# bittremieux/falcon

Hardware: AMD Instinct MI355X
Metric: spectra clustered/sec @1/2/4/8 GPU; cosine-kernel HBM GB/s vs roofline (higher is better)
Workload: dtype f32; 1 GPU; one dataset of 1000000 synthetic spectra (1000000 per GPU; charges 2+3; precursor m/z 400-1200), low_dim=400, n_neighbors=64, n_neighbors_ann=128, n_probe=16, eps=0.1, precursor_tol=20ppm, mz_interval=1.0, batch_size=32768; exchange=none, parallelism=1 GPU

## Files before the change

### falcon_amd/csrc/common.h

```cpp
#pragma once
#include <hip/hip_runtime.h>
#include <stdint.h>
#include <stdio.h>
#include <string.h>
#include <string>
#include <vector>
#include "../../include/falcon_hip.h"

namespace fal {

void set_error(const char* fmt, ...);

#define FAL_CHECK_HIP(expr)                                                          \
    do {                                                                             \
        hipError_t _e = (expr);                                                      \
        if (_e != hipSuccess) {                                                      \
            fal::set_error("%s:%d: %s failed: %s", __FILE__, __LINE__, #expr,        \
                           hipGetErrorString(_e));                                   \
            return (_e == hipErrorOutOfMemory) ? FAL_ENOMEM : FAL_EHIP;              \
        }                                                                            \
    } while (0)

#define FAL_REQUIRE(cond, code, ...)                                                 \
    do {                                                                             \
        if (!(cond)) {                                                               \
            fal::set_error(__VA_ARGS__);                                             \
            return (code);                                                           \
        }                                                                            \
    } while (0)

#define FAL_TRY(expr)                                                                \
    do {                                                                             \
        int _r = (expr);                                                             \
        if (_r != FAL_OK) return _r;                                                 \
    } while (0)

constexpr int kNumStages = 9;
constexpr int kNumSlots = 37;
enum Stage { ST_VECTORIZE = 0, ST_BUILD = 1, ST_COARSE = 2, ST_SCAN = 3, ST_SELECT = 4,
             ST_FILTER = 5, ST_DBSCAN = 6, ST_TAIL = 7,
             ST_KERNEL = 8 };

struct Scratch {
    void* ptr = nullptr;
    size_t cap = 0;
};

}

struct fal_ctx {
    int device = -1;
    hipStream_t stream = nullptr;
    bool own_stream = false;
    void* pinned = nullptr;
    size_t pinned_cap = 0;
    int pinned_reserve(size_t bytes, void** out);
    unsigned char* arena = nullptr;
    size_t arena_off = 0;
    int upload(void* dst, const void* src, size_t bytes);
    int num_cus = 256;
    int persistent_wgs = 256;
    bool timing = false;
    struct StageTimer {
        std::vector<std::pair<hipEvent_t, hipEvent_t>> ev;
        size_t used = 0;
    } timers[fal::kNumStages];
    fal::Scratch scratch[fal::kNumSlots];
    int32_t* fb_host = nullptr;
    int32_t* zero_dev = nullptr;
    int64_t counters[10] = {0, 0, 0, 0, 0, 0, 0, 0, 0, 0};

    struct PoolBlock { void* ptr; size_t cap; bool used; };
    std::vector<PoolBlock> pool;
    int pool_alloc(size_t bytes, void** out);
    void pool_free(void* ptr);

    bool debug_poison = false;
    int call_depth = 0;
    uint64_t call_epoch = 1;
    uint64_t slot_epoch[fal::kNumSlots] = {};
    uint32_t slot_gen[fal::kNumSlots] = {};
    std::vector<void*> retired;
    std::vector<bool> retired_held;
    void release_retired();
    int reserve(int slot, size_t bytes, void** out);
    void release(int slot) { slot_epoch[slot] = 0; }
    void stage_reset(int stage);
    int stage_begin(int stage, hipEvent_t* stop_out, hipStream_t on = nullptr);
    int stage_end(hipEvent_t stop, hipStream_t on = nullptr);
};

namespace fal {

struct StageScope {
    fal_ctx* c;
    hipEvent_t stop = nullptr;
    bool on;
    hipStream_t s;
    StageScope(fal_ctx* ctx, int stage, hipStream_t stream = nullptr, bool enable = true)
        : c(ctx), on(ctx->timing && enable), s(stream) {
        if (on) c->stage_begin(stage, &stop, s);
    }
    ~StageScope() {
        if (on && stop) c->stage_end(stop, s);
    }
};

struct CallScope {
    fal_ctx* c;
    explicit CallScope(fal_ctx* ctx) : c(ctx) {
        if (c && c->call_depth++ == 0) {
            ++c->call_epoch;
            if (!c->retired.empty()) c->release_retired();
        }
    }
    ~CallScope() {
        if (c) --c->call_depth;
    }
};

static inline int64_t ceil_div(int64_t a, int64_t b) { return (a + b - 1) / b; }
// ... 89 lines not shown
```

### falcon_amd/csrc/ivf.h

```cpp
#pragma once
#include <vector>
#include "common.h"

namespace fal {
constexpr int kSparseW = 64;
constexpr uint16_t kColPad = 0xFFFF;
constexpr uint16_t kColDense = 0xFFFE;

enum { SLOT_JOBS = 0, SLOT_SIMS = 1, SLOT_PROBES = 2, SLOT_PROBE_SIM = 3, SLOT_QOFF = 4, SLOT_JOBS2 = 5,
       SLOT_MISC = 6, SLOT_MISC2 = 7, SLOT_SORT = 8, SLOT_SORT2 = 9, SLOT_TAIL = 10, SLOT_TAIL2 = 11,
       SLOT_TAIL3 = 12, SLOT_TAIL4 = 13, SLOT_DB = 14, SLOT_DB2 = 15, SLOT_DB3 = 16, SLOT_FIN = 17, SLOT_FIN2 = 18,
       SLOT_FIN3 = 19, SLOT_INV = 20, SLOT_INVCNT = 21, SLOT_SIMS2 = 22, SLOT_TILEJOB = 23, SLOT_FUSED = 24, SLOT_FUSED2 = 25, SLOT_FUSED3 = 26, SLOT_JOBS3 = 27, SLOT_WIN = 28, SLOT_CURSORS = 29, SLOT_ITEMS = 30,
       SLOT_EXACT = 31, SLOT_EXACT2 = 32, SLOT_EXACT3 = 33, SLOT_EXACT4 = 34, SLOT_EXACT5 = 35, SLOT_EXACT6 = 36 };
int launch_exclusive_scan(fal_ctx* ctx, const int64_t* in, int64_t n, int64_t* out);
}
struct fal_ivf;
namespace fal {
int ivf_ensure_xl(fal_ctx* ctx, const fal_ivf* ivf);
}

struct fal_ivf {
    fal_ctx* ctx = nullptr;
    int64_t n = 0;
    int d = 0;
    const float* X = nullptr;
    const float* Xl = nullptr;
    float* Xl_owned = nullptr;
    const void* X16 = nullptr;
    int x16_planes = 0;
    const void* Xpre = nullptr;
    int rows_signed = 0;
    int rows_f16 = 0;
    int32_t* neg_dev = nullptr;
    const void* X16pre = nullptr;
    int32_t* pos_of_row = nullptr;
    int ckeys_stride = 0;
    uint16_t* ckeys = nullptr;
    std::vector<int64_t> bucket_off;
    std::vector<int32_t> n_list;
    std::vector<int64_t> list_base;
    int64_t total_lists = 0;
    int n_ivf_buckets = 0;
    int64_t ivf_waves = 0;
    float* centroids = nullptr;
    int32_t* assign = nullptr;
    int32_t* perm = nullptr;
    uint16_t* sp_cols = nullptr;
    float* sp_vals = nullptr;
    uint16_t* sq16 = nullptr;
    int rows_many = 0;
    int64_t* list_off = nullptr;
    int64_t* counts = nullptr;
    void* bk_dev = nullptr;
};
```

### falcon_amd/csrc/scan.h

```cpp
#pragma once
#include "common.h"
#include "simtile.h"

namespace fal {

enum { EPI_STORE = 0, EPI_ARGMAX = 1 };
enum { MODE_DENSE = 0, MODE_IVF = 1 };

constexpr size_t kSimsSlack = 2048;

struct SelectArgs {
    const float* sims;
    int64_t sims_base;
    int k;
    float* out_sim;
    int32_t* out_idx;
    const DenseJob* jobs;
    int n_jobs;
    int64_t tile_begin;
    const int32_t* tile_job;
    int ids_are_rows;
    int n_probe;
    const int32_t* probes;
    const int64_t* list_off;
    const int64_t* q_sim_off;
    const int32_t* perm;
    const float* f_pmz;
    const float* f_rt;
    double f_tol, f_rt_tol;
    int f_is_da;
    int f_keep;
    int32_t* nb_idx;
    float* nb_dist;
    int32_t* nb_count;
};

bool dense4_supports(int d);
int launch_dense4(fal_ctx* ctx, const float* X, int d, const DenseJob* jobs, const DenseJob* jobs_host, int n_jobs, float* sims,
                  int64_t sims_base);
bool dense4ab_supports(int d);
int launch_dense4ab(fal_ctx* ctx, const float* X, int d, const DenseJob* jobs, const DenseJob* jobs_host, int n_jobs, float* sims,
                    int64_t sims_base);
int launch_dense_tiny4(fal_ctx* ctx, const float* X, int d, const DenseJob* jobs, int n_jobs, float* sims, int64_t sims_base);
int launch_flat_exact_small(fal_ctx* ctx, const float* X, int d, const DenseJob* jobs, int n_jobs, float* sims, int64_t sims_base);
int launch_dense(fal_ctx* ctx, int stage, int epi, const float* Q, const float* Cm, int d, const DenseJob* jobs,
                 int n_jobs, int64_t tile_begin, int64_t n_tiles, float* sims, int64_t sims_base, int32_t* assign,
                 int64_t xcd_list_tiles = 0);
constexpr int kAssignSeg = 2048;
constexpr int kAssignGroup = 128;
constexpr int kAssignMergeLists = 2048;
struct AssignJob {
    int64_t row0;
    int64_t cent0;
    int32_t nrows;
    int32_t ncent;
    int32_t id_base;
    int32_t part0;
};
int launch_assign(fal_ctx* ctx, int stage, const float* X, const float* centroids, int d, const AssignJob* jobs, int64_t n_jobs,
                  int64_t n_wave_jobs, int64_t n, unsigned long long* keys, int32_t* assign);
bool assign16_supports(int d);
int launch_cvt_f16(fal_ctx* ctx, const float* in, void* out, int64_t count);
int launch_assign16(fal_ctx* ctx, int stage, const void* X16, const float* X, const void* C16, const float* Cn, int d,
                    const AssignJob* jobs, int64_t n_single, int64_t n_merge, int64_t n_group, int64_t n_rows, int32_t* assign,
                    uint16_t* ckeys = nullptr, int ckeys_stride = 0, const uint16_t* sp_cols = nullptr,
                    const float* sp_vals = nullptr, int merge_max_lists = 4 * kAssignGroup, int64_t merge_rows = 0);
struct ListScanArgs {
    const float* Xl;
    int d;
    const int64_t* list_off;
    const int64_t* inv_off;
    const int64_t* ltile_off;
    int group_shift;
    const int32_t* inv_q;
    const int64_t* inv_dest;
    int64_t list_begin, list_end;
    int64_t tile_begin, n_tiles_max;
    float* sims;
    int64_t sims_base;
    float* sink;
};
int launch_list_scan(fal_ctx* ctx, const ListScanArgs& a);
int launch_select(fal_ctx* ctx, int stage, int mode, const SelectArgs& a, int64_t n_blocks, hipStream_t on = nullptr);
int launch_scan16(fal_ctx* ctx, int planes, const void* Xs, int d, const DenseJob* jobs, int n_jobs, int64_t list_tiles,
                  float* sims, int64_t sims_base, float* sink);

}
```

### falcon_amd/csrc/scan.hip

```cpp
#include <math.h>
#include <stdlib.h>
#include <string.h>
#include <algorithm>
#include "common.h"
#include "simtile.h"
#include "scan.h"
#include "select.h"
#include "ivf.h"

namespace fal {

template <int DH4, int EPI>
__global__ __launch_bounds__(64, 1) void dense_kernel(
    const float* __restrict__ Q, const float* __restrict__ Cm, int d, const DenseJob* __restrict__ jobs,
    int n_jobs, int64_t tile_begin, int64_t n_tiles, float* __restrict__ sims, int64_t sims_base,
    int32_t* __restrict__ assign, int xcd_lists, int symmetric) {
    DenseJob job;
    int lt;
    int ji = 0;
    if (xcd_lists) {
        if (!find_job_xcd(jobs, n_jobs, blockIdx.x, &ji, &lt)) return;
        job = jobs[ji];
    } else {
        const int64_t per_xcd = (n_tiles + 7) / 8;
        const int64_t lt_all = (int64_t)(blockIdx.x & 7) * per_xcd + (blockIdx.x >> 3);
        if ((blockIdx.x >> 3) >= per_xcd || lt_all >= n_tiles) return;
        const int64_t t = tile_begin + lt_all;
        job = jobs[find_job(jobs, n_jobs, t)];
        lt = (int)(t - job.tile0);
    }
    const int lane = threadIdx.x, r = lane & 31, h = lane >> 5;
    const int nq_t = min(32, job.nq - 32 * lt);
    const int dh = d >> 1, dh4 = dh >> 2;

    float q[DH4 * 4];
    {
        const int64_t qrow = job.q_row0 + 32 * (int64_t)lt + min(r, nq_t - 1);
        load_half_row<DH4>(q, Q + qrow * d + (int64_t)h * dh, dh4);
    }
    float best = -INFINITY;
    int bestc = 0x7fffffff;
    const int nc = job.nc;
    float* out = nullptr;
    const int ncp = (nc + 31) & ~31;
    if (EPI == EPI_STORE) out = sims + (job.obase - sims_base) + (int64_t)(32 * lt) * ncp + r;

    const int c_first = (EPI == EPI_STORE && symmetric) ? 32 * lt : 0;
    float* outT = nullptr;
    if (EPI == EPI_STORE && symmetric) outT = sims + (job.obase - sims_base) + (int64_t)r * ncp + 32 * lt + 4 * h;
    const int c_last = ((nc - 1) >> 5) << 5;
    constexpr bool kDown = EPI == EPI_STORE;
    const int c_begin = kDown ? c_last : 0, c_step = kDown ? -32 : 32;
    const int n_chunks = (c_last - c_first) / 32 + 1;
    CandStream<DH4> cs;
    const float* cur = Cm + (job.c_row0 + min(c_begin + r, nc - 1)) * d + (int64_t)h * dh;
    cs.prime(cur, dh4);
    f32x16 prev;
    int prev_c0 = c_begin;
#pragma unroll
    for (int i = 0; i < 16; ++i) prev[i] = (EPI == EPI_STORE) ? 0.f : -INFINITY;
    auto epilogue = [&]() {
        if (EPI == EPI_STORE) {
#pragma unroll
            for (int i = 0; i < 16; ++i) out[mfma32_row(i, h) * ncp + prev_c0] = prev[i];
            if (symmetric) {
                float* t = outT + (int64_t)prev_c0 * ncp;
#pragma unroll
                for (int g = 0; g < 4; ++g)
                    *reinterpret_cast<float4*>(t + 8 * g) = make_float4(prev[4 * g], prev[4 * g + 1], prev[4 * g + 2], prev[4 * g + 3]);
                __builtin_amdgcn_sched_group_barrier(0x040, 20, 0);
            } else {
                __builtin_amdgcn_sched_group_barrier(0x040, 16, 0);
            }
        } else {
#pragma unroll
            for (int i = 0; i < 16; ++i) {
                const int c = prev_c0 + mfma32_row(i, h);
                const float s = prev[i];
                if (c < nc && s > best) {
                    best = s;
                    bestc = c;
                }
            }
        }
    };
    for (int ci = 0, c0 = c_begin; ci < n_chunks; ++ci, c0 += c_step) {
        const float* nxt = Cm + (job.c_row0 + min(max(c0 + c_step, 0) + r, nc - 1)) * d + (int64_t)h * dh;
        const f32x16 acc = (EPI == EPI_STORE) ? cs.template dot<true>(q, cur, nxt, dh4, epilogue)
                                              : cs.template dot<false>(q, cur, nxt, dh4, epilogue);
// ... 148 lines not shown
#pragma unroll
                    for (int k = j * kDmaPer; k < (j + 1) * kDmaPer && k < kPieces; ++k) issue_piece(k, next);
                }
            } else {
#pragma unroll
                for (int k = (j - kHalf) * kStPer; k < (j - kHalf + 1) * kStPer && k < kStores; ++k) store_piece(k);
                __builtin_amdgcn_sched_group_barrier(0x040, kStPer, 0);
            }
        }
        asm volatile("s_nop 15\n\ts_nop 7" : "+a"(acc));
        prev = acc;
        prev_c0 = c0;
    };
    auto take_queries = [&](const unsigned char* lb) {
#pragma unroll
        for (int j = 0; j < DH4; ++j) {
            float4 v = make_float4(0.f, 0.f, 0.f, 0.f);
            if (j < dh4) v = *reinterpret_cast<const float4*>(lb + 16 * j);
            q[4 * j + 0] = v.x;
            q[4 * j + 1] = v.y;
            q[4 * j + 2] = v.z;
            q[4 * j + 3] = v.w;
        }
    };

    int after = 0;
    if (preloaded) after = prev_stored ? 2 * kStores : 0;
    else issue(Target{rows, nc, c_first, par ? buf1 : buf0, true});
    bool odd = par != 0;
    int ci = 0, c0 = c_first;
    for (;;) {
        if (!odd) {
            chunk_barrier(after);
            Target next = ci + 1 < n_chunks ? Target{rows, nc, c0 + 32, buf1, true} : first_of_next;
            next.buf = buf1;
            if (active && c0 == c_stop) {
                if (MODE == 2) load_init(c0);
                take_queries(my0);
            }
            if (active && c0 >= c_stop) {
                compute(my0, c0, next);
                after = kStores;
            } else {
                if (next.valid) issue(next);
                after = 0;
            }
            ++ci;
            c0 += 32;
            if (ci >= n_chunks) break;
        }
        odd = false;
        chunk_barrier(after);
        Target next = ci + 1 < n_chunks ? Target{rows, nc, c0 + 32, buf0, true} : first_of_next;
        next.buf = buf0;
        if (active && c0 == c_stop) {
            if (MODE == 2) load_init(c0);
            take_queries(my1);
        }
        if (active && c0 >= c_stop) {
            compute(my1, c0, next);
            after = kStores;
        } else {
            if (next.valid) issue(next);
            after = 0;
        }
        ++ci;
        c0 += 32;
        if (ci >= n_chunks) break;
    }
    if (active) epilogue();
    if (tid == 0) next_item = fetched;
    asm volatile("s_waitcnt lgkmcnt(0)\n\ts_barrier ; dma-ok: cursor hand-off only" ::: "memory");
    const int nxt2 = next_item;
    par = (par + n_chunks) & 1;
    preloaded = have_next;
    prev_stored = active;
    cur = nxt;
    nxt = nxt2;
    }
    }
}

template <int DH4>
__global__ __launch_bounds__(256, 1) void dense_tiny4_kernel(const float* __restrict__ X, int d, const DenseJob* __restrict__ jobs,
                                                             int n_jobs, float* __restrict__ sims, int64_t sims_base,
                                                             int32_t* __restrict__ cursor) {
    extern __shared__ __attribute__((aligned(16))) unsigned char stream_lds[];
    __shared__ int32_t next_item;
    const int tid = threadIdx.x, w = tid >> 6, lane = tid & 63, r = lane & 31, h = lane >> 5;
    const int dh = d >> 1, dh4 = dh >> 2;
    const int row_bytes = d * 4, rs = row_bytes + 16;
    constexpr int kParts = (DH4 * 32 + 1023) / 1024;
    const uint32_t lds0 = (uint32_t)(size_t)(__attribute__((address_space(3))) const void*)stream_lds;
    for (;;) {
        __syncthreads();
        if (tid == 0) next_item = atomicAdd(cursor, 1);
        __syncthreads();
        const int j0 = 4 * next_item;
        if (j0 >= n_jobs) break;
        const bool active = j0 + w < n_jobs;
        float q[DH4 * 4];
#pragma unroll
        for (int round = 0; round < 2; ++round) {
            if (round) __syncthreads();
            const int jb = j0 + 2 * round + (w >> 1);
            if (jb < n_jobs) {
                const int64_t row0 = jobs[jb].c_row0;
                const int nb = jobs[jb].nq;
#pragma unroll
                for (int p = 0; p < kParts; ++p) {
                    if (p * 1024 + lane * 16 < row_bytes) {
#pragma unroll
                        for (int i = 0; i < 16; ++i) {
                            const int sr = 16 * w + i;
                            const unsigned char* src = reinterpret_cast<const unsigned char*>(X + (row0 + min(sr & 31, nb - 1)) * d) +
                                                       p * 1024 + lane * 16;
                            const uint32_t l = (uint32_t)__builtin_amdgcn_readfirstlane((int)(lds0 + (uint32_t)(sr * rs + p * 1024)));
                            asm volatile("s_mov_b32 m0, %1\n\ts_nop 0\n\tglobal_load_lds_dwordx4 %0, off" ::"v"(src), "s"(l) : "memory", "m0");
                        }
                    }
                }
            }
            asm volatile("s_waitcnt vmcnt(0)\n\ts_barrier" ::: "memory");
            if ((w >> 1) == round && active) {
                const unsigned char* lb = stream_lds + ((w & 1) * 32 + r) * rs + h * (dh * 4);
#pragma unroll
                for (int j = 0; j < DH4; ++j) {
                    float4 v = make_float4(0.f, 0.f, 0.f, 0.f);
                    if (j < dh4) v = *reinterpret_cast<const float4*>(lb + 16 * j);
                    q[4 * j + 0] = v.x;
                    q[4 * j + 1] = v.y;
                    q[4 * j + 2] = v.z;
                    q[4 * j + 3] = v.w;
                }
            }
        }
        if (!active) continue;
        const DenseJob job = jobs[j0 + w];
        f32x16 acc;
#pragma unroll
        for (int i = 0; i < 16; ++i) acc[i] = 0.f;
#pragma unroll
        for (int j = 0; j < DH4 * 4; ++j) acc = __builtin_amdgcn_mfma_f32_32x32x2f32(q[j], q[j], acc, 0, 0, 0);
        asm volatile("s_nop 15\n\ts_nop 7" : "+a"(acc));
        float* const out = sims + (job.obase - sims_base) + r;
#pragma unroll
        for (int i = 0; i < 16; ++i) out[mfma32_row(i, h) * 32] = acc[i];
    }
}


bool dense4_supports(int d) { return d % 8 == 0 && d >= 32 && (d <= 400 || (d > 512 && d <= 800 && d % 16 == 0)); }

int launch_dense4(fal_ctx* ctx, const float* X, int d, const DenseJob* jobs, const DenseJob* jobs_host, int n_jobs, float* sims,
                  int64_t sims_base) {
    if (n_jobs <= 0) return FAL_OK;
    {
        const char* e = getenv("FALCON_DENSE4");
        if (e && !strcmp(e, "ab") && dense4ab_supports(d)) return launch_dense4ab(ctx, X, d, jobs, jobs_host, n_jobs, sims, sims_base);
    }
    const bool split = d > 512;
    const int dv = split ? d / 2 : d;
    const int dh4 = dv / 8;
    std::vector<int32_t> table(16, 0);
    for (int x = 0; x < 8; ++x) {
        for (int j = x; j < n_jobs; j += 8)
            for (int g = 0; g < (jobs_host[j].nq + 127) / 128; ++g) {
                table.push_back(j);
                table.push_back(g);
            }
        table[x + 1] = (int32_t)((table.size() - 16) / 2);
    }
    const int64_t n_items = table[8];
    int32_t* table_dev = nullptr;
    FAL_TRY(ctx->reserve(SLOT_ITEMS, sizeof(int32_t) * table.size(), (void**)&table_dev));
    FAL_TRY(ctx->upload(table_dev, table.data(), sizeof(int32_t) * table.size()));
    const size_t lds = (size_t)2 * 32 * (dv * 4 + 16);
    int32_t* cursors = nullptr;
    FAL_TRY(ctx->reserve(SLOT_CURSORS, sizeof(int32_t) * 16, (void**)&cursors));
    dim3 grid((unsigned)std::min<int64_t>(n_items, ctx->persistent_wgs)), block(256);
    StageScope ts(ctx, ST_SCAN);
    StageScope tk(ctx, ST_KERNEL);
#define FAL_LAUNCH_DENSE4(DH4, MODE, KOFF)                                                                          \
    do {                                                                                                            \
        FAL_CHECK_HIP(hipMemsetAsync(cursors, 0, sizeof(int32_t) * 8, ctx->stream));                                \
        FAL_CHECK_HIP(hipFuncSetAttribute((const void*)dense4_kernel<DH4, MODE>, hipFuncAttributeMaxDynamicSharedMemorySize, \
                                          (int)lds));                                                               \
        hipLaunchKernelGGL((dense4_kernel<DH4, MODE>), grid, block, lds, ctx->stream, X, dv, KOFF, jobs, sims, sims_base, cursors, \
                           table_dev);                                                                              \
    } while (0)
    if (split) {
        if (dh4 > 50 || d % 16 != 0) {
            set_error("dense4 supports low_dim <= 400 and 513..800 in steps of 16 (got %d)", d);
            return FAL_EUNSUPPORTED;
        }
        FAL_LAUNCH_DENSE4(50, 1, 0);
        FAL_LAUNCH_DENSE4(50, 2, dv / 2);
    } else if (dh4 <= 8) FAL_LAUNCH_DENSE4(8, 0, 0);
    else if (dh4 <= 16) FAL_LAUNCH_DENSE4(16, 0, 0);
    else if (dh4 <= 32) FAL_LAUNCH_DENSE4(32, 0, 0);
    else if (dh4 <= 50) FAL_LAUNCH_DENSE4(50, 0, 0);
    else {
        set_error("dense4 supports low_dim <= 400 and 513..800 in steps of 16 (got %d)", d);
        return FAL_EUNSUPPORTED;
    }
#undef FAL_LAUNCH_DENSE4
    FAL_CHECK_HIP(hipGetLastError());
    return FAL_OK;
}

__global__ __launch_bounds__(64) void flat_exact_small_kernel(const float* __restrict__ X, int d, const DenseJob* __restrict__ jobs,
                                                              int n_jobs, float* __restrict__ sims, int64_t sims_base) {
    const int lane = threadIdx.x;
    for (int j = blockIdx.x; j < n_jobs; j += gridDim.x) {
        const DenseJob job = jobs[j];
        const int nc = job.nc, W = (nc + 31) & ~31;
        float* const out = sims + (job.obase - sims_base);
        for (int i = 0; i < job.nq; ++i)
            for (int c = lane; c < nc; c += 64)
                out[(int64_t)(i >> 5) * 32 * W + (i & 31) * W + c] = exact_dot(X + (job.q_row0 + i) * (int64_t)d, X + (job.c_row0 + c) * (int64_t)d, d);
    }
}

int launch_flat_exact_small(fal_ctx* ctx, const float* X, int d, const DenseJob* jobs, int n_jobs, float* sims, int64_t sims_base) {
    if (n_jobs <= 0) return FAL_OK;
    StageScope ts(ctx, ST_SCAN);
    hipLaunchKernelGGL(flat_exact_small_kernel, dim3((unsigned)std::min<int64_t>(n_jobs, (int64_t)ctx->num_cus * 16)), dim3(64), 0,
                       ctx->stream, X, d, jobs, n_jobs, sims, sims_base);
    FAL_CHECK_HIP(hipGetLastError());
    return FAL_OK;
}

int launch_dense_tiny4(fal_ctx* ctx, const float* X, int d, const DenseJob* jobs, int n_jobs, float* sims, int64_t sims_base) {
    if (n_jobs <= 0) return FAL_OK;
    const int dh4 = d / 8;
    const size_t lds = (size_t)2 * 32 * (d * 4 + 16);
    int32_t* cursors = nullptr;
    FAL_TRY(ctx->reserve(SLOT_CURSORS, sizeof(int32_t) * 16, (void**)&cursors));
    cursors += 8;
    dim3 grid((unsigned)std::min<int64_t>(ceil_div(n_jobs, 4), ctx->persistent_wgs)), block(256);
    StageScope ts(ctx, ST_SCAN);
    FAL_CHECK_HIP(hipMemsetAsync(cursors, 0, sizeof(int32_t), ctx->stream));
#define FAL_LAUNCH_TINY4(DH4)                                                                                       \
    do {                                                                                                            \
        FAL_CHECK_HIP(hipFuncSetAttribute((const void*)dense_tiny4_kernel<DH4>, hipFuncAttributeMaxDynamicSharedMemorySize, \
                                          (int)lds));                                                               \
        hipLaunchKernelGGL((dense_tiny4_kernel<DH4>), grid, block, lds, ctx->stream, X, d, jobs, n_jobs, sims, sims_base, \
                           cursors);                                                                                \
    } while (0)
    if (dh4 <= 8) FAL_LAUNCH_TINY4(8);
    else if (dh4 <= 16) FAL_LAUNCH_TINY4(16);
    else if (dh4 <= 32) FAL_LAUNCH_TINY4(32);
    else if (dh4 <= 50) FAL_LAUNCH_TINY4(50);
    else {
        set_error("dense_tiny4 supports low_dim <= 400 (got %d)", d);
        return FAL_EUNSUPPORTED;
    }
#undef FAL_LAUNCH_TINY4
    FAL_CHECK_HIP(hipGetLastError());
    return FAL_OK;
}

template <int EPI>
static int launch_dense_t(fal_ctx* ctx, int stage, const float* Q, const float* Cm, int d, const DenseJob* jobs,
                          int n_jobs, int64_t tile_begin, int64_t n_tiles, float* sims, int64_t sims_base,
                          int32_t* assign, int64_t xcd_list_tiles) {
    if (n_tiles <= 0) return FAL_OK;
    const int symmetric = (EPI == EPI_STORE && xcd_list_tiles > 0 && Q == Cm) ? 1 : 0;
    const int dh4 = d / 8;
    const int xcd_lists = xcd_list_tiles > 0;
    const int64_t per_xcd = xcd_lists ? xcd_list_tiles : (n_tiles + 7) / 8;
    FAL_REQUIRE(per_xcd * 8 < (int64_t)INT32_MAX, FAL_EUNSUPPORTED, "too many tiles in one launch");
 dim3 grid((unsigned)(per_xcd * 8)), block(64);
    StageScope ts(ctx, stage);
    StageScope tk(ctx, ST_KERNEL, nullptr, stage == ST_SCAN);
#define FAL_LAUNCH_DENSE(DH4)                                                                              \
    hipLaunchKernelGGL((dense_kernel<DH4, EPI>), grid, block, 0, ctx->stream, Q, Cm, d, jobs, n_jobs,      \
                       tile_begin, n_tiles, sims, sims_base, assign, xcd_lists, symmetric)
    if (dh4 <= 8) FAL_LAUNCH_DENSE(8);
    else if (dh4 <= 16) FAL_LAUNCH_DENSE(16);
    else if (dh4 <= 32) FAL_LAUNCH_DENSE(32);
    else if (dh4 <= 50) FAL_LAUNCH_DENSE(50);
    else if (dh4 <= 64) FAL_LAUNCH_DENSE(64);
    else {
        set_error("float32 scan supports low_dim <= 512 (got %d)", d);
        return FAL_EUNSUPPORTED;
    }
#undef FAL_LAUNCH_DENSE
    FAL_CHECK_HIP(hipGetLastError());
    return FAL_OK;
}

int launch_dense(fal_ctx* ctx, int stage, int epi, const float* Q, const float* Cm, int d, const DenseJob* jobs,
                 int n_jobs, int64_t tile_begin, int64_t n_tiles, float* sims, int64_t sims_base, int32_t* assign,
                 int64_t xcd_list_tiles) {
    if (epi == EPI_STORE)
        return launch_dense_t<EPI_STORE>(ctx, stage, Q, Cm, d, jobs, n_jobs, tile_begin, n_tiles, sims, sims_base,
                                         assign, xcd_list_tiles);
    return launch_dense_t<EPI_ARGMAX>(ctx, stage, Q, Cm, d, jobs, n_jobs, tile_begin, n_tiles, sims, sims_base, assign,
                                      xcd_list_tiles);
}

template <int MODE, bool FUSE>
__global__ __launch_bounds__(64) __attribute__((amdgpu_waves_per_eu(MODE == MODE_DENSE ? 8 : 3, 8))) void select_kernel(SelectArgs a) {
    __shared__ uint32_t sel_u[kSelBuf];
    __shared__ uint32_t sel_id[kSelBuf];
    __shared__ int64_t seg_off[FAL_MAX_N_PROBE + 1];
    __shared__ int64_t seg_src[FAL_MAX_N_PROBE];
    const int lane = threadIdx.x;
    const int k = a.k;
    const unsigned qblock = blockIdx.x;

    SelQuery qy{nullptr, 0, 0};
    int64_t out_row = 0;
    const int64_t t = a.tile_begin + (qblock >> 5);
    const int ql = qblock & 31;
    const DenseJob job = a.jobs[a.tile_job[qblock >> 5]];
    const int lt = (int)(t - job.tile0);
    if (32 * lt + ql >= job.nq) return;
    if (MODE == MODE_DENSE) {
        qy.nc = job.nc;
        qy.row = a.sims + (job.obase - a.sims_base) + (int64_t)(32 * lt + ql) * ((job.nc + 31) & ~31);
        out_row = job.q_row0 + 32 * (int64_t)lt + ql;
        qy.id0 = a.ids_are_rows ? job.c_row0 : 0;
    } else {
        const int64_t p = job.q_row0 + 32 * (int64_t)lt + ql;
        const int np = a.n_probe;
        const int32_t* pr = a.probes + p * np;
        const int64_t lbase = job.c_row0;
        if (lane == 0) {
            int64_t off = 0;
// ... 77 lines not shown
```

### falcon_amd/csrc/search.hip

```cpp
#include <algorithm>
#include <stdlib.h>
#include <string.h>
#include "common.h"
#include "scan.h"
#include "ivf.h"
#include "util.h"
#include "fused.h"
#include "ivf16.h"
#include "coarse16.h"

namespace fal {

template <int NPV>
__global__ void probe_totals_kernel(const int32_t* __restrict__ probes, int np, const DenseJob* __restrict__ jobs,
                                    int n_jobs, int64_t n_tiles, const int64_t* __restrict__ list_off,
                                    int64_t* __restrict__ totals) {
    const int64_t g = blockIdx.x * (int64_t)blockDim.x + threadIdx.x;
    const int64_t t = g >> 5;
    int64_t tot = 0;
    if (t < n_tiles) {
        const DenseJob job = jobs[find_job(jobs, n_jobs, t)];
        const int lt = (int)(t - job.tile0), ql = (int)(g & 31);
        if (32 * lt + ql < job.nq) {
            const int64_t p = job.q_row0 + 32 * (int64_t)lt + ql;
// ... 373 lines not shown
                xt32[x] += tiles;
            }
            flat.push_back({row0, row0, cur.floats, cur.tiles, (int32_t)nb, (int32_t)nb, xtile0});
            cur.tiles += tiles;
            cur.floats += floats;
            cur.j1++;
        }
        close();
    }
    int64_t ivf_tiles = 0, coarse_o = 0;
    int max_n_list = 0;
    for (int64_t b = 0; b < n_buckets; ++b) {
        const int64_t row0 = ivf->bucket_off[b], nb = ivf->bucket_off[b + 1] - row0;
        if (nb == 0 || ivf->n_list[b] == 1) continue;
        const int64_t tiles = ceil_div(nb, 32);
        coarse.push_back({row0, ivf->list_base[b], coarse_o, ivf_tiles, (int32_t)nb, ivf->n_list[b], 0});
        ivf_tiles += tiles;
        coarse_o += tiles * 32 * (((int64_t)ivf->n_list[b] + 31) & ~31ll);
        max_n_list = std::max(max_n_list, ivf->n_list[b]);
    }
    auto make_batches = [&](const std::vector<DenseJob>& jobs, int64_t n_tiles, std::vector<int64_t>& cuts, size_t& need) {
        cuts.assign(1, 0);
        need = 0;
        int64_t used = 0;
        for (const DenseJob& j : jobs) {
            const int64_t tiles = ceil_div(j.nq, 32), per_tile = 32 * (((int64_t)j.nc + 31) & ~31ll);
            for (int64_t t = 0; t < tiles;) {
                int64_t room = ((int64_t)cap - used) / per_tile;
                if (room <= 0 && used > 0) {
                    cuts.push_back(j.tile0 + t);
                    used = 0;
                    continue;
                }
                if (room <= 0) room = 1;
                const int64_t take = std::min(room, tiles - t);
                used += take * per_tile;
                need = std::max(need, (size_t)used);
                t += take;
            }
        }
        if (cuts.back() != n_tiles) cuts.push_back(n_tiles);
    };
    auto obase_of_tile = [&](const std::vector<DenseJob>& jobs, int64_t t) -> int64_t {
        size_t lo = 0, hi = jobs.size() - 1;
        while (lo < hi) {
            size_t mid = (lo + hi + 1) / 2;
            if (jobs[mid].tile0 <= t) lo = mid; else hi = mid - 1;
        }
        return jobs[lo].obase + (t - jobs[lo].tile0) * 32 * (((int64_t)jobs[lo].nc + 31) & ~31ll);
    };

    std::vector<int64_t> coarse_cuts;
    size_t need_coarse = 0;
    if (!coarse.empty()) make_batches(coarse, ivf_tiles, coarse_cuts, need_coarse);

    DenseJob *flat_dev = nullptr, *coarse_dev = nullptr;
    if (!flat.empty()) {
        FAL_TRY(ctx->reserve(SLOT_JOBS, sizeof(DenseJob) * flat.size(), (void**)&flat_dev));
        FAL_TRY(ctx->upload(flat_dev, flat.data(), sizeof(DenseJob) * flat.size()));
    }
    if (!coarse.empty()) {
        FAL_TRY(ctx->reserve(SLOT_JOBS2, sizeof(DenseJob) * coarse.size(), (void**)&coarse_dev));
        FAL_TRY(ctx->upload(coarse_dev, coarse.data(), sizeof(DenseJob) * coarse.size()));
    }
    float* sims = nullptr;
    const size_t sims_floats = std::max(need_flat, need_coarse);
    FAL_TRY(ctx->reserve(SLOT_SIMS, sizeof(float) * (sims_floats + kSimsSlack), (void**)&sims));
    for (size_t bi = 0; bi < flat_batches.size(); ++bi) {
        const FlatBatch& fb = flat_batches[bi];
        float* buf = sims;
        const DenseJob* jb = flat_dev + fb.j0;
        const int nj = (int)(fb.j1 - fb.j0);
        if (fb.jm > fb.j0)
            FAL_TRY(launch_scan16(ctx, ivf->x16_planes, ivf->X16, d, jb, (int)(fb.jm - fb.j0), fb.list_tiles16, buf, 0,
                                  buf + sims_floats));
        if (fb.js > fb.jm)
            FAL_TRY(launch_dense4(ctx, ivf->X, d, flat_dev + fb.jm, flat.data() + fb.jm, (int)(fb.js - fb.jm), buf, 0));
        if (fb.jk > fb.js)
            FAL_TRY(launch_dense(ctx, ST_SCAN, EPI_STORE, ivf->X, ivf->X, d, flat_dev + fb.js, (int)(fb.jk - fb.js), 0, fb.tiles, buf, 0,
                                 nullptr, fb.list_tiles1));
        if (fb.j1 > fb.jk && d > 512)
            FAL_TRY(launch_flat_exact_small(ctx, ivf->X, d, flat_dev + fb.jk, (int)(fb.j1 - fb.jk), buf, 0));
        else if (fb.j1 > fb.jk && have4)
            FAL_TRY(launch_dense_tiny4(ctx, ivf->X, d, flat_dev + fb.jk, (int)(fb.j1 - fb.jk), buf, 0));
        else if (fb.j1 > fb.jk)
            FAL_TRY(launch_dense(ctx, ST_SCAN, EPI_STORE, ivf->X, ivf->X, d, flat_dev + fb.jk, (int)(fb.j1 - fb.jk), 0,
                                 fb.tiles, buf, 0, nullptr, fb.list_tiles32));
        SelectArgs sa{};
        sa.sims = buf; sa.sims_base = 0; sa.k = k_ann; sa.out_sim = sim; sa.out_idx = idx;
        sa.jobs = jb; sa.n_jobs = nj; sa.tile_begin = 0; sa.ids_are_rows = 1;
        set_filter(sa, nf);
        FAL_TRY(launch_select(ctx, ST_SELECT, MODE_DENSE, sa, fb.tiles * 32));
    }
    if (!fused) {
        ctx->counters[0] = 0;
        ctx->counters[4] = 0;
    }
    for (const FlatBatch& fb : flat_batches)
        for (size_t j = fb.j0; j < fb.j1; ++j) {
            const int64_t ch = ceil_div(flat[j].nc, 32);
            ctx->counters[4] += 1024 * (ch * (ch + 1) / 2);
        }
    for (const DenseJob& j : flat) ctx->counters[0] += (int64_t)j.nq * j.nc;
    ctx->counters[7] = ctx->counters[8] = 0;
    if (have4)
        for (const FlatBatch& fb : flat_batches)
            for (size_t j = fb.jk; j < fb.j1; ++j) {
                ctx->counters[7] += (int64_t)flat[j].nq * flat[j].nc;
                ctx->counters[8] += 1024;
            }
    ctx->counters[1] = 0;
    if (!fused) {
        ctx->counters[2] = (int64_t)flat_batches.size();
        ctx->counters[3] = (int64_t)(sizeof(float) * std::max(need_flat, need_coarse));
    }
    if (coarse.empty()) return FAL_OK;
    for (const DenseJob& j : coarse) ctx->counters[1] += (int64_t)j.nq * j.nc;

    const int np = std::min(n_probe, max_n_list);
    int32_t* probes = nullptr;
    float* probe_sim = nullptr;
    int64_t *totals = nullptr, *q_sim_off = nullptr;
    FAL_TRY(ctx->reserve(SLOT_PROBES, sizeof(int32_t) * (size_t)ivf->n * np, (void**)&probes));
    FAL_TRY(ctx->reserve(SLOT_PROBE_SIM, sizeof(float) * (size_t)ivf->n * np, (void**)&probe_sim));
    const int64_t n_slots = ivf_tiles * 32;
    FAL_TRY(ctx->reserve(SLOT_QOFF, sizeof(int64_t) * (size_t)(n_slots + 1), (void**)&q_sim_off));
    FAL_TRY(ctx->reserve(SLOT_MISC, sizeof(int64_t) * (size_t)(n_slots + 2), (void**)&totals));
    FAL_CHECK_HIP(hipMemsetAsync(totals, 0, sizeof(int64_t) * (size_t)(n_slots + 2), st));
    const bool from_keys = ivf->ckeys != nullptr && ivf->X != nullptr &&
                           (ivf->ckeys_stride <= 512 || (ivf->ckeys_stride <= 2048 && ivf->sp_cols != nullptr));
    if (from_keys) {
        Coarse16Args ca{ivf->ckeys, ivf->ckeys_stride, ivf->X, ivf->centroids, d, coarse_dev, (int)coarse.size(), ivf_tiles, nullptr,
                        ivf->perm, np, probes};
        ca.sp_cols = ivf->sp_cols;
        ca.sp_vals = ivf->sp_vals;
        FAL_TRY(launch_coarse16(ctx, ca));
    }
    if (!from_keys) FAL_TRY(ivf_ensure_xl(ctx, ivf));
    for (size_t bi = 0; !from_keys && bi + 1 < coarse_cuts.size(); ++bi) {
        const int64_t t0 = coarse_cuts[bi], t1 = coarse_cuts[bi + 1];
        const int64_t base = obase_of_tile(coarse, t0);
        FAL_TRY(launch_dense(ctx, ST_COARSE, EPI_STORE, ivf->Xl, ivf->centroids, d, coarse_dev, (int)coarse.size(), t0,
                             t1 - t0, sims, base, nullptr));
        SelectArgs sa{};
        sa.sims = sims; sa.sims_base = base; sa.k = np; sa.out_sim = probe_sim; sa.out_idx = probes;
        sa.jobs = coarse_dev; sa.n_jobs = (int)coarse.size(); sa.tile_begin = t0; sa.ids_are_rows = 0;
        FAL_TRY(launch_select(ctx, ST_COARSE, MODE_DENSE, sa, (t1 - t0) * 32));
    }
    const bool fused_totals = max_n_list <= 4096;
    if (!fused_totals) {
        StageScope ts(ctx, ST_COARSE);
        const dim3 tg((unsigned)ceil_div(n_slots, 256));
        if (np == 16)
            hipLaunchKernelGGL(probe_totals_kernel<4>, tg, dim3(256), 0, st, probes, np, coarse_dev, (int)coarse.size(), ivf_tiles,
                               ivf->list_off, totals);
        else if (np == 32)
            hipLaunchKernelGGL(probe_totals_kernel<8>, tg, dim3(256), 0, st, probes, np, coarse_dev, (int)coarse.size(), ivf_tiles,
                               ivf->list_off, totals);
        else
            hipLaunchKernelGGL(probe_totals_kernel<0>, tg, dim3(256), 0, st, probes, np, coarse_dev, (int)coarse.size(), ivf_tiles,
                               ivf->list_off, totals);
        FAL_TRY(device_scan_i64(ctx, totals, n_slots, q_sim_off, SLOT_MISC2));
    }
    const int group_shift = 7;
    const int64_t TL = ivf->total_lists;
    const int64_t n_pairs_max = ivf->n * (int64_t)np;
    int32_t *cnt = nullptr, *inv_q = nullptr;
// ... 206 lines not shown
```

Baseline: 195.3 million spectra/s.

## Pack small buckets into 32-row tiles and pipeline tiny4 kernel per wave

The tiny-bucket dense kernel now bin-packs many small buckets (size up to 32 rows) into shared 32-row MFMA tiles on the host. Previously each bucket took a whole 32x32 tile and padded rows were computed. The kernel becomes a single-wave workgroup that software-pipelines pack loads into LDS via global_load_lds, prefetching pack words and job metadata ahead. Output is masked to the diagonal block of each bucket. In exchange it adds host-side packing and an upload per launch, plus a more fragile pipeline that mixes a ticket counter with static striding.

```diff
diff --git a/falcon_amd/csrc/common.h b/falcon_amd/csrc/common.h
--- a/falcon_amd/csrc/common.h
+++ b/falcon_amd/csrc/common.h
@@ -36,7 +36,7 @@
     } while (0)
 
 constexpr int kNumStages = 9;
-constexpr int kNumSlots = 37;
+constexpr int kNumSlots = 38;
 enum Stage { ST_VECTORIZE = 0, ST_BUILD = 1, ST_COARSE = 2, ST_SCAN = 3, ST_SELECT = 4,
              ST_FILTER = 5, ST_DBSCAN = 6, ST_TAIL = 7,
              ST_KERNEL = 8 };
diff --git a/falcon_amd/csrc/flatplan.h b/falcon_amd/csrc/flatplan.h
--- /dev/null
+++ b/falcon_amd/csrc/flatplan.h
@@ -0,0 +1,42 @@
+#pragma once
+#include <stdint.h>
+#include <vector>
+
+namespace fal {
+
+constexpr int kPackRows = 32;
+constexpr int kPackJobBits = 26;
+
+template <class Job>
+inline int build_tiny_packs(const Job* jobs, int n_jobs, std::vector<int32_t>& words) {
+    words.clear();
+    std::vector<int32_t> by_size[kPackRows + 1];
+    int64_t rows = 0;
+    for (int j = 0; j < n_jobs; ++j)
+        if (jobs[j].nq > 0 && jobs[j].nq <= kPackRows) {
+            by_size[jobs[j].nq].push_back(j);
+            rows += jobs[j].nq;
+        }
+    words.reserve((size_t)(rows + rows / 8 + 2 * kPackRows));
+    size_t next[kPackRows + 1] = {};
+    int largest = kPackRows, n_packs = 0;
+    for (;;) {
+        while (largest > 0 && next[largest] == by_size[largest].size()) --largest;
+        if (largest == 0) break;
+        const size_t at = words.size();
+        words.resize(at + kPackRows, -1);
+        int used = 0;
+        for (int s = largest; s > 0; --s) {
+            while (next[s] < by_size[s].size() && used + s <= kPackRows) {
+                const int j = by_size[s][next[s]++];
+                for (int i = 0; i < s; ++i) words[at + used + i] = (int32_t)(((uint32_t)j << 5) | (uint32_t)used);
+                used += s;
+            }
+            if (s > kPackRows - used) s = kPackRows - used + 1;
+        }
+        ++n_packs;
+    }
+    return n_packs;
+}
+
+}
diff --git a/falcon_amd/csrc/ivf.h b/falcon_amd/csrc/ivf.h
--- a/falcon_amd/csrc/ivf.h
+++ b/falcon_amd/csrc/ivf.h
@@ -11,7 +11,8 @@
        SLOT_MISC = 6, SLOT_MISC2 = 7, SLOT_SORT = 8, SLOT_SORT2 = 9, SLOT_TAIL = 10, SLOT_TAIL2 = 11,
        SLOT_TAIL3 = 12, SLOT_TAIL4 = 13, SLOT_DB = 14, SLOT_DB2 = 15, SLOT_DB3 = 16, SLOT_FIN = 17, SLOT_FIN2 = 18,
        SLOT_FIN3 = 19, SLOT_INV = 20, SLOT_INVCNT = 21, SLOT_SIMS2 = 22, SLOT_TILEJOB = 23, SLOT_FUSED = 24, SLOT_FUSED2 = 25, SLOT_FUSED3 = 26, SLOT_JOBS3 = 27, SLOT_WIN = 28, SLOT_CURSORS = 29, SLOT_ITEMS = 30,
-       SLOT_EXACT = 31, SLOT_EXACT2 = 32, SLOT_EXACT3 = 33, SLOT_EXACT4 = 34, SLOT_EXACT5 = 35, SLOT_EXACT6 = 36 };
+       SLOT_EXACT = 31, SLOT_EXACT2 = 32, SLOT_EXACT3 = 33, SLOT_EXACT4 = 34, SLOT_EXACT5 = 35, SLOT_EXACT6 = 36,
+       SLOT_PACKS = 37 };
 int launch_exclusive_scan(fal_ctx* ctx, const int64_t* in, int64_t n, int64_t* out);
 }
 struct fal_ivf;
diff --git a/falcon_amd/csrc/scan.h b/falcon_amd/csrc/scan.h
--- a/falcon_amd/csrc/scan.h
+++ b/falcon_amd/csrc/scan.h
@@ -41,7 +41,8 @@
 bool dense4ab_supports(int d);
 int launch_dense4ab(fal_ctx* ctx, const float* X, int d, const DenseJob* jobs, const DenseJob* jobs_host, int n_jobs, float* sims,
                     int64_t sims_base);
-int launch_dense_tiny4(fal_ctx* ctx, const float* X, int d, const DenseJob* jobs, int n_jobs, float* sims, int64_t sims_base);
+int launch_dense_tiny4(fal_ctx* ctx, const float* X, int d, const DenseJob* jobs, const DenseJob* jobs_host, int n_jobs, float* sims,
+                       int64_t sims_base);
 int launch_flat_exact_small(fal_ctx* ctx, const float* X, int d, const DenseJob* jobs, int n_jobs, float* sims, int64_t sims_base);
 int launch_dense(fal_ctx* ctx, int stage, int epi, const float* Q, const float* Cm, int d, const DenseJob* jobs,
                  int n_jobs, int64_t tile_begin, int64_t n_tiles, float* sims, int64_t sims_base, int32_t* assign,
diff --git a/falcon_amd/csrc/scan.hip b/falcon_amd/csrc/scan.hip
--- a/falcon_amd/csrc/scan.hip
+++ b/falcon_amd/csrc/scan.hip
@@ -5,6 +5,7 @@
 #include "common.h"
 #include "simtile.h"
 #include "scan.h"
+#include "flatplan.h"
 #include "select.h"
 #include "ivf.h"
 
@@ -319,70 +320,114 @@
 }
 
 template <int DH4>
-__global__ __launch_bounds__(256, 1) void dense_tiny4_kernel(const float* __restrict__ X, int d, const DenseJob* __restrict__ jobs,
-                                                             int n_jobs, float* __restrict__ sims, int64_t sims_base,
-                                                             int32_t* __restrict__ cursor) {
+__global__ __launch_bounds__(64) void dense_tiny4_kernel(const float* __restrict__ X, int d, const DenseJob* __restrict__ jobs,
+                                                         const int32_t* __restrict__ packs, int n_packs, float* __restrict__ sims,
+                                                         int64_t sims_base, int32_t* __restrict__ cursor) {
     extern __shared__ __attribute__((aligned(16))) unsigned char stream_lds[];
-    __shared__ int32_t next_item;
-    const int tid = threadIdx.x, w = tid >> 6, lane = tid & 63, r = lane & 31, h = lane >> 5;
+    const int lane = threadIdx.x, r = lane & 31, h = lane >> 5;
     const int dh = d >> 1, dh4 = dh >> 2;
     const int row_bytes = d * 4, rs = row_bytes + 16;
     constexpr int kParts = (DH4 * 32 + 1023) / 1024;
     const uint32_t lds0 = (uint32_t)(size_t)(__attribute__((address_space(3))) const void*)stream_lds;
-    for (;;) {
-        __syncthreads();
-        if (tid == 0) next_item = atomicAdd(cursor, 1);
-        __syncthreads();
-        const int j0 = 4 * next_item;
-        if (j0 >= n_jobs) break;
-        const bool active = j0 + w < n_jobs;
-        float q[DH4 * 4];
-#pragma unroll
-        for (int round = 0; round < 2; ++round) {
-            if (round) __syncthreads();
-            const int jb = j0 + 2 * round + (w >> 1);
-            if (jb < n_jobs) {
-                const int64_t row0 = jobs[jb].c_row0;
-                const int nb = jobs[jb].nq;
+    const int G = (int)gridDim.x;
+
+    struct PackLane {
+        const float* src;
+        float* out;
+        int o, nb;
+    };
+    auto word_of = [&](int p) { return packs[(int64_t)min(p, n_packs - 1) * kPackRows + r]; };
+    struct JobLane { int64_t c_row0, obase; int nq; };
+    auto fetch = [&](int word, int p) {
+        JobLane J{0, 0, 0};
+        if (p < n_packs && word >= 0) {
+            const DenseJob* jb = jobs + (word >> 5);
+            J = JobLane{jb->c_row0, jb->obase, jb->nq};
+        }
+        return J;
+    };
+    auto resolve = [&](int word, const JobLane& J) {
+        PackLane L{X, sims, 0, 0};
+        if (J.nq > 0) {
+            L.o = word & 31;
+            L.nb = J.nq;
+            L.src = X + (J.c_row0 + (r - L.o)) * d;
+            L.out = sims + (J.obase - sims_base);
+        }
+        return L;
+    };
+    auto issue = [&](const PackLane& L) {
+        const int n_rows = __popcll(__ballot(L.nb > 0)) >> 1;
+        const uint64_t mine = (uint64_t)(size_t)L.src;
+#pragma unroll
+        for (int i = 0; i < kPackRows; ++i) {
+            if (i < n_rows) {
+                const uint64_t row = (uint64_t)(uint32_t)__builtin_amdgcn_readlane((int)(uint32_t)mine, i) |
+                                     ((uint64_t)(uint32_t)__builtin_amdgcn_readlane((int)(uint32_t)(mine >> 32), i) << 32);
 #pragma unroll
                 for (int p = 0; p < kParts; ++p) {
                     if (p * 1024 + lane * 16 < row_bytes) {
-#pragma unroll
-                        for (int i = 0; i < 16; ++i) {
-                            const int sr = 16 * w + i;
-                            const unsigned char* src = reinterpret_cast<const unsigned char*>(X + (row0 + min(sr & 31, nb - 1)) * d) +
-                                                       p * 1024 + lane * 16;
-                            const uint32_t l = (uint32_t)__builtin_amdgcn_readfirstlane((int)(lds0 + (uint32_t)(sr * rs + p * 1024)));
-                            asm volatile("s_mov_b32 m0, %1\n\ts_nop 0\n\tglobal_load_lds_dwordx4 %0, off" ::"v"(src), "s"(l) : "memory", "m0");
-                        }
+                        const unsigned char* src = reinterpret_cast<const unsigned char*>((size_t)row) + p * 1024 + lane * 16;
+                        const uint32_t l = (uint32_t)__builtin_amdgcn_readfirstlane((int)(lds0 + (uint32_t)(i * rs + p * 1024)));
+                        asm volatile("s_mov_b32 m0, %1\n\ts_nop 0\n\tglobal_load_lds_dwordx4 %0, off" ::"v"(src), "s"(l) : "memory", "m0");
                     }
                 }
             }
-            asm volatile("s_waitcnt vmcnt(0)\n\ts_barrier" ::: "memory");
-            if ((w >> 1) == round && active) {
-                const unsigned char* lb = stream_lds + ((w & 1) * 32 + r) * rs + h * (dh * 4);
-#pragma unroll
-                for (int j = 0; j < DH4; ++j) {
-                    float4 v = make_float4(0.f, 0.f, 0.f, 0.f);
-                    if (j < dh4) v = *reinterpret_cast<const float4*>(lb + 16 * j);
-                    q[4 * j + 0] = v.x;
-                    q[4 * j + 1] = v.y;
-                    q[4 * j + 2] = v.z;
-                    q[4 * j + 3] = v.w;
-                }
-            }
-        }
-        if (!active) continue;
-        const DenseJob job = jobs[j0 + w];
+        }
+    };
+    auto ticket = [&]() {
+        int t = 0;
+        if (lane == 0) t = (int)atomicInc(reinterpret_cast<unsigned*>(cursor), 0xFFFFFFFFu);
+        return t;
+    };
+
+    int p0 = (int)blockIdx.x, p1 = p0 + G, p2 = p1 + G;
+    if (p0 >= n_packs) return;
+    const int w0 = word_of(p0), w1 = word_of(p1);
+    PackLane L0 = resolve(w0, fetch(w0, p0));
+    issue(L0);
+    PackLane L1 = resolve(w1, fetch(w1, p1));
+    int w2 = word_of(p2);
+    int t3 = p2 + G - 4 * G;
+    while (p0 < n_packs) {
+        asm volatile("s_waitcnt vmcnt(0)" ::: "memory");
+        asm volatile("" : "+v"(w2), "+v"(t3));
+        float q[DH4 * 4];
+        {
+            const unsigned char* lb = stream_lds + r * rs + h * (dh * 4);
+#pragma unroll
+            for (int j = 0; j < DH4; ++j) {
+                float4 v = make_float4(0.f, 0.f, 0.f, 0.f);
+                if (j < dh4) v = *reinterpret_cast<const float4*>(lb + 16 * j);
+                q[4 * j + 0] = v.x;
+                q[4 * j + 1] = v.y;
+                q[4 * j + 2] = v.z;
+                q[4 * j + 3] = v.w;
+            }
+        }
+        asm volatile("s_waitcnt lgkmcnt(0)" ::: "memory");
+        if (p1 < n_packs) issue(L1);
+        const JobLane J2 = fetch(w2, p2);
+        const int p3 = __builtin_amdgcn_readfirstlane(t3) + 4 * G;
+        const int w3 = word_of(p3);
+        const int t4 = ticket();
+        __builtin_amdgcn_sched_barrier(0);
         f32x16 acc;
 #pragma unroll
         for (int i = 0; i < 16; ++i) acc[i] = 0.f;
 #pragma unroll
         for (int j = 0; j < DH4 * 4; ++j) acc = __builtin_amdgcn_mfma_f32_32x32x2f32(q[j], q[j], acc, 0, 0, 0);
         asm volatile("s_nop 15\n\ts_nop 7" : "+a"(acc));
-        float* const out = sims + (job.obase - sims_base) + r;
-#pragma unroll
-        for (int i = 0; i < 16; ++i) out[mfma32_row(i, h) * 32] = acc[i];
+        __builtin_amdgcn_sched_barrier(0);
+#pragma unroll
+        for (int i = 0; i < 16; ++i) {
+            const int row = mfma32_row(i, h) - L0.o;
+            if (row >= 0 && row < L0.nb) L0.out[row * 32 + (r - L0.o)] = acc[i];
+        }
+        p0 = p1; L0 = L1;
+        p1 = p2; L1 = resolve(w2, J2);
+        p2 = p3; w2 = w3;
+        t3 = t4;
     }
 }
 
@@ -468,22 +513,34 @@
     return FAL_OK;
 }
 
-int launch_dense_tiny4(fal_ctx* ctx, const float* X, int d, const DenseJob* jobs, int n_jobs, float* sims, int64_t sims_base) {
+int launch_dense_tiny4(fal_ctx* ctx, const float* X, int d, const DenseJob* jobs, const DenseJob* jobs_host, int n_jobs, float* sims,
+                       int64_t sims_base) {
     if (n_jobs <= 0) return FAL_OK;
+    FAL_REQUIRE(n_jobs < (1 << kPackJobBits), FAL_EUNSUPPORTED, "too many one-block buckets in one launch");
+    for (int j = 0; j < n_jobs; ++j)
+        FAL_REQUIRE(jobs_host[j].nq <= kPackRows, FAL_EINTERNAL, "dense_tiny4: a bucket of %d rows", (int)jobs_host[j].nq);
     const int dh4 = d / 8;
-    const size_t lds = (size_t)2 * 32 * (d * 4 + 16);
+    std::vector<int32_t> words;
+    const int n_packs = build_tiny_packs(jobs_host, n_jobs, words);
+    if (n_packs <= 0) return FAL_OK;
+    int32_t* packs_dev = nullptr;
+    ctx->release(SLOT_PACKS);
+    FAL_TRY(ctx->reserve(SLOT_PACKS, sizeof(int32_t) * words.size(), (void**)&packs_dev));
+    FAL_TRY(ctx->upload(packs_dev, words.data(), sizeof(int32_t) * words.size()));
+    const size_t lds = (size_t)kPackRows * (d * 4 + 16);
     int32_t* cursors = nullptr;
     FAL_TRY(ctx->reserve(SLOT_CURSORS, sizeof(int32_t) * 16, (void**)&cursors));
     cursors += 8;
-    dim3 grid((unsigned)std::min<int64_t>(ceil_div(n_jobs, 4), ctx->persistent_wgs)), block(256);
+    const int64_t per_cu = std::min<int64_t>(4, (160 * 1024) / (int64_t)lds);
+    dim3 grid((unsigned)std::min<int64_t>(n_packs, per_cu * ctx->persistent_wgs)), block(64);
     StageScope ts(ctx, ST_SCAN);
     FAL_CHECK_HIP(hipMemsetAsync(cursors, 0, sizeof(int32_t), ctx->stream));
 #define FAL_LAUNCH_TINY4(DH4)                                                                                       \
     do {                                                                                                            \
         FAL_CHECK_HIP(hipFuncSetAttribute((const void*)dense_tiny4_kernel<DH4>, hipFuncAttributeMaxDynamicSharedMemorySize, \
                                           (int)lds));                                                               \
-        hipLaunchKernelGGL((dense_tiny4_kernel<DH4>), grid, block, lds, ctx->stream, X, d, jobs, n_jobs, sims, sims_base, \
-                           cursors);                                                                                \
+        hipLaunchKernelGGL((dense_tiny4_kernel<DH4>), grid, block, lds, ctx->stream, X, d, jobs, packs_dev, n_packs, sims, \
+                           sims_base, cursors);                                                                     \
     } while (0)
     if (dh4 <= 8) FAL_LAUNCH_TINY4(8);
     else if (dh4 <= 16) FAL_LAUNCH_TINY4(16);
diff --git a/falcon_amd/csrc/search.hip b/falcon_amd/csrc/search.hip
--- a/falcon_amd/csrc/search.hip
+++ b/falcon_amd/csrc/search.hip
@@ -479,7 +479,7 @@
         if (fb.j1 > fb.jk && d > 512)
             FAL_TRY(launch_flat_exact_small(ctx, ivf->X, d, flat_dev + fb.jk, (int)(fb.j1 - fb.jk), buf, 0));
         else if (fb.j1 > fb.jk && have4)
-            FAL_TRY(launch_dense_tiny4(ctx, ivf->X, d, flat_dev + fb.jk, (int)(fb.j1 - fb.jk), buf, 0));
+            FAL_TRY(launch_dense_tiny4(ctx, ivf->X, d, flat_dev + fb.jk, flat.data() + fb.jk, (int)(fb.j1 - fb.jk), buf, 0));
         else if (fb.j1 > fb.jk)
             FAL_TRY(launch_dense(ctx, ST_SCAN, EPI_STORE, ivf->X, ivf->X, d, flat_dev + fb.jk, (int)(fb.j1 - fb.jk), 0,
                                  fb.tiles, buf, 0, nullptr, fb.list_tiles32));
```

Result: no change. 194.4 million spectra/s (-0.5%).
